# luoao-kddi/SCP

Hardware: AMD Instinct MI355X
Metric: KITTI frames/sec encode (SCP-EHEM, level 16) + bpp match vs ref (higher is better)
Workload: dtype f32 (dense layers and attention as bf16x3 split on bf16 MFMA, feature kNN as f16x3 split on f16 MFMA, fp32 accumulate; position kNN / CDF in fp32); 1 GPU; SCP-EHEM KITTI-like synthetic 120k-pt frames, --spher --mullevel lidar_level=16 (BASELINE.json configs[2]), seeded random weights; nodes_per_frame=577403, windows_per_frame=100, frames_per_gpu=46, frames_in_flight=4, frames_per_launch_sequence=1, transform=host-numpy on a prefetch thread (strict identity: the reference's integers), parallelism=frame-sharded x1, rank_cores=256, rank_cores_pinned=False

## Files before the change

scp_amd/build.py:

```python
import os
import subprocess
import sys

HERE = os.path.dirname(os.path.abspath(__file__))
CSRC = os.path.join(HERE, "csrc")
LIB = os.path.join(HERE, "libscp_hip.so")
SOURCES = ["api.cpp", "geom.hip", "sort_u64.hip", "cdf.hip", "rangecoder.cpp", "legacy_octree.cpp",
           "knn.hip", "edge.hip", "attn.hip", "octattn.hip", "octattn_f16.hip", "octattn_embed.hip", "octattn_rowinv.hip", "gemm.hip", "gemm_split.hip", "rowchain.hip", "fused.hip", "metrics.hip", "plan.hip"]
HIPCC = os.environ.get("HIPCC", "/opt/rocm/bin/hipcc")
FLAGS = ["-O3", "--offload-arch=gfx950", "-fPIC", "-std=c++17", "-Wall", "-Wno-unused-function",
         "-Wno-unused-result", "-fvisibility=hidden", "-x", "hip"]


EXTRA = {"geom.hip": ["-ffp-contract=off"], "knn.hip": ["-ffp-contract=off"], "cdf.hip": ["-ffp-contract=off"],
         "edge.hip": ["-ffp-contract=off"], "metrics.hip": ["-ffp-contract=off"], "octattn_embed.hip": ["-ffp-contract=off"],
         "octattn_rowinv.hip": ["-ffp-contract=off"]}
if os.environ.get("SCP_ATTN_DEFS"):
    EXTRA["attn.hip"] = os.environ["SCP_ATTN_DEFS"].split()
if os.environ.get("SCP_KNN_DEFS"):
    EXTRA["knn.hip"] = EXTRA["knn.hip"] + os.environ["SCP_KNN_DEFS"].split()
if os.environ.get("SCP_RC_DEFS"):
    EXTRA["rowchain.hip"] = os.environ["SCP_RC_DEFS"].split()


def _stale(target, deps):
    if not os.path.exists(target):
        return True
    t = os.path.getmtime(target)
    return any(os.path.getmtime(d) > t for d in deps)


def build(force=False, verbose=False):
    srcs = [os.path.join(CSRC, s) for s in SOURCES if os.path.exists(os.path.join(CSRC, s))]
    hdrs = [os.path.join(CSRC, f) for f in os.listdir(CSRC) if f.endswith(".h")] + [os.path.join(HERE, "..", "include", "scp.h")]
    objs = []
    os.makedirs(os.path.join(CSRC, "build"), exist_ok=True)
    procs = []
    for s in srcs:
        o = os.path.join(CSRC, "build", os.path.basename(s) + ".o")
        objs.append(o)
        cmd = [HIPCC] + FLAGS + EXTRA.get(os.path.basename(s), []) + ["-c", s, "-o", o]
        stamp, line = o + ".cmd", " ".join(cmd)
        same_cmd = os.path.exists(stamp) and open(stamp).read() == line
        if force or not same_cmd or _stale(o, [s] + hdrs):
            for stale in (stamp, o):
                if os.path.exists(stale):
                    os.remove(stale)
            if verbose:
                print(" ".join(cmd), file=sys.stderr)
            procs.append((s, subprocess.Popen(cmd), stamp, line))
    bad = []
    for s, p, stamp, line in procs:
        if p.wait() != 0:
            bad.append(s)
            continue
        with open(stamp, "w") as f:
            f.write(line)
    if bad:
        raise RuntimeError("hipcc failed for: " + ", ".join(bad))
    if force or procs or _stale(LIB, objs):
        cmd = [HIPCC, "--offload-arch=gfx950", "-shared", "-fPIC", "-o", LIB] + objs
        if verbose:
            print(" ".join(cmd), file=sys.stderr)
        subprocess.check_call(cmd)
    return LIB


if __name__ == "__main__":
    print(build(force="--force" in sys.argv, verbose=True))
```

scp_amd/csrc/rowchain.hip:

```cpp
#include <stdlib.h>
#include "scp_internal.h"

typedef __bf16 rbf16x8 __attribute__((ext_vector_type(8)));
typedef float rf32x16 __attribute__((ext_vector_type(16)));
typedef float rf32x4 __attribute__((ext_vector_type(4)));
typedef int ri32x4 __attribute__((ext_vector_type(4)));
typedef __attribute__((address_space(3))) void *rc_lds_ptr_t;
typedef const __attribute__((address_space(1))) void *rc_glb_ptr_t;

#define RC_ROWS 128
#define RC_SLOT 32768
#define RC_RING (4 * RC_SLOT)
#define RC_BOUNCE 4096
#define RC_OFF_BOUNCE RC_RING
#define RC_OFF_BIAS (RC_RING + 4 * RC_BOUNCE)
#define RC_LDS (RC_OFF_BIAS + 16384)

__device__ __forceinline__ void rc_dma16(const void *g, char *l) {
    __builtin_amdgcn_global_load_lds((rc_glb_ptr_t)g, (rc_lds_ptr_t)l, 16, 0, 0);
}

typedef float rf32x2 __attribute__((ext_vector_type(2)));
typedef __bf16 rbf16x2 __attribute__((ext_vector_type(2)));
typedef unsigned ru32x4 __attribute__((ext_vector_type(4)));
typedef unsigned ru32x2 __attribute__((ext_vector_type(2)));
__device__ __forceinline__ unsigned rc_pack2(float a, float b) {
    const rf32x2 v = {a, b};
    return __builtin_bit_cast(unsigned, __builtin_convertvector(v, rbf16x2));
}
__device__ __forceinline__ void rc_split2(float a, float b, unsigned &hi, unsigned &lo) {
    asm volatile("" : "+v"(a), "+v"(b));
    hi = rc_pack2(a, b);
    lo = rc_pack2(a - __builtin_bit_cast(float, hi << 16), b - __builtin_bit_cast(float, hi & 0xffff0000u));
}
__device__ __forceinline__ void rc_split8(const float *f, rbf16x8 &hi, rbf16x8 &lo) {
    ru32x4 h, l;
#pragma unroll
    for (int i = 0; i < 4; ++i) { unsigned a, b; rc_split2(f[2 * i], f[2 * i + 1], a, b); h[i] = a; l[i] = b; }
    hi = __builtin_bit_cast(rbf16x8, h);
    lo = __builtin_bit_cast(rbf16x8, l);
}

struct RcLane {
    int lane, col, h, w;
    int frag;
    int rg;
};

__device__ __forceinline__ RcLane rc_lane() {
    RcLane L;
    const int tid = threadIdx.x;
    L.lane = tid & 63; L.col = L.lane & 31; L.h = L.lane >> 5;
    L.w = __builtin_amdgcn_readfirstlane(tid >> 6);
    L.frag = (L.col & 15) * 64 + ((L.h ^ ((L.col >> 2) & 3)) << 4);
    L.rg = L.col >> 4;
    return L;
}

__device__ __forceinline__ void rc_issue_rowchunk(const RcLane &L, const __bf16 *Whi, const __bf16 *Wlo, int g, char *slot) {
#pragma unroll
    for (int j = 0; j < 4; ++j) {
        const int p = L.w + 4 * j;
        const int64_t off = ((int64_t)g * 16 + p) * 512 + L.lane * 8;
        rc_dma16(Whi + off, slot + p * 1024);
        rc_dma16(Wlo + off, slot + 16384 + p * 1024);
    }
}

__device__ __forceinline__ void rc_issue_kchunk(const RcLane &L, const __bf16 *Whi, const __bf16 *Wlo, int c, int nks, char *slot) {
#pragma unroll
    for (int j = 0; j < 4; ++j) {
        const int p = L.w + 4 * j;
        const int64_t off = ((int64_t)p * nks + c) * 512 + L.lane * 8;
        rc_dma16(Whi + off, slot + p * 1024);
        rc_dma16(Wlo + off, slot + 16384 + p * 1024);
    }
}

__device__ __forceinline__ rbf16x8 rc_frag_rowchunk(const RcLane &L, const char *slot, int plane, int s) {
    return *(const rbf16x8 *)(slot + plane * 16384 + (L.rg * 8 + (s >> 1)) * 1024 + (L.frag ^ ((s & 1) << 5)));
}

__device__ __forceinline__ rbf16x8 rc_frag_kchunk(const RcLane &L, const char *slot, int plane, int b, int t) {
    return *(const rbf16x8 *)(slot + plane * 16384 + (2 * b + L.rg) * 1024 + (L.frag ^ (t << 5)));
}

#define RC_DS_READ4_WAIT(d0, a0, o0, d1, a1, o1, d2, a2, o2, d3, a3, o3)                                                              \
    asm volatile("ds_read_b128 %0, %4 offset:%8\n\tds_read_b128 %1, %5 offset:%9\n\tds_read_b128 %2, %6 offset:%10\n\t"                   \
                 "ds_read_b128 %3, %7 offset:%11\n\ts_waitcnt lgkmcnt(0)"                                                              \
                 : "=&v"(d0), "=&v"(d1), "=&v"(d2), "=&v"(d3) : "v"(a0), "v"(a1), "v"(a2), "v"(a3), "n"(o0), "n"(o1), "n"(o2), "n"(o3) : "memory")
#define RC_DS_READ(dst, addr, off) asm volatile("ds_read_b128 %0, %1 offset:%2" : "=v"(dst) : "v"(addr), "n"(off) : "memory")

__device__ __forceinline__ void rc_mfma3x2(rf32x16 &c0, rf32x16 &c1, const rbf16x8 &a0h, const rbf16x8 &a0l, const rbf16x8 &a1h,
                                           const rbf16x8 &a1l, const rbf16x8 &bh, const rbf16x8 &bl) {
    c0 = __builtin_amdgcn_mfma_f32_32x32x16_bf16(a0l, bh, c0, 0, 0, 0);
    c1 = __builtin_amdgcn_mfma_f32_32x32x16_bf16(a1l, bh, c1, 0, 0, 0);
    c0 = __builtin_amdgcn_mfma_f32_32x32x16_bf16(a0h, bl, c0, 0, 0, 0);
    c1 = __builtin_amdgcn_mfma_f32_32x32x16_bf16(a1h, bl, c1, 0, 0, 0);
    c0 = __builtin_amdgcn_mfma_f32_32x32x16_bf16(a0h, bh, c0, 0, 0, 0);
    c1 = __builtin_amdgcn_mfma_f32_32x32x16_bf16(a1h, bh, c1, 0, 0, 0);
}

__device__ __forceinline__ void rc_store_block(const RcLane &L, char *bounce, const rf32x4 v[4], __amdgpu_buffer_rsrc_t rs, int ldo_bytes, int voff,
                                               int ch0) {
#pragma unroll
    for (int q = 0; q < 4; ++q)
        *(rf32x4 *)(bounce + L.col * 128 + (((2 * q + L.h) ^ (L.col & 7)) << 4)) = v[q];
    asm volatile("s_waitcnt lgkmcnt(0)" ::: "memory");
    rf32x4 y[4];
#pragma unroll
    for (int it = 0; it < 4; ++it) {
        const int rho = 8 * it + (L.lane >> 3), kap = L.lane & 7;
        y[it] = *(const rf32x4 *)(bounce + rho * 128 + ((kap ^ (rho & 7)) << 4));
    }
#pragma unroll
    for (int it = 0; it < 4; ++it) __builtin_amdgcn_raw_buffer_store_b128(__builtin_bit_cast(ri32x4, y[it]), rs, voff, it * 8 * ldo_bytes + ch0 * 4, 0);
    asm volatile("s_waitcnt lgkmcnt(0)" ::: "memory");
}

__device__ __forceinline__ void rc_ln_stats(const float *v , float eps, float &mean, float &rstd) {
    float s = 0.f;
#pragma unroll
    for (int i = 0; i < 128; i += 4) s += (v[i] + v[i + 1]) + (v[i + 2] + v[i + 3]);
    s += __shfl_xor(s, 32);
    mean = s * (1.0f / 256.0f);
    float q = 0.f;
#pragma unroll
    for (int i = 0; i < 128; ++i) { const float d = v[i] - mean; q += d * d; }
    q += __shfl_xor(q, 32);
    rstd = rsqrtf(q * (1.0f / 256.0f) + eps);
}

struct RcLnLinArgs {
    const float *x; int64_t ldx;
    const float *valid;
    const __bf16 *Whi, *Wlo;
    const float *bias, *wbeta;
    float *out; int64_t ldo;
    int M, N;
    float eps;
    int probe;
    unsigned long long *dbg;
    __bf16 *planes; int64_t plane_bytes; int nq;
    int ngroups;
};

#define RC_DS_WRITE(addr, val, off) asm volatile("ds_write_b128 %0, %1 offset:%2" :: "v"(addr), "v"(val), "n"(off) : "memory")

#define RC_SB __builtin_amdgcn_sched_barrier(0)
#ifndef RC_SKEW
#define RC_SKEW 0
#endif
#if RC_SKEW > 0
#define RC_STEP_BARRIER(WAITS, w)                                                                                                          \
    do {                                                                                                                                   \
        int _rc_n;                                                                                                                         \
        asm volatile("s_waitcnt " WAITS "\n\ts_barrier\n\ts_mov_b32 %0, %1\n\ts_cmp_eq_u32 %0, 0\n\ts_cbranch_scc1 .Lrcskew_done%=\n"          \
                     ".Lrcskew_loop%=:\n\ts_nop 7\n\ts_sub_u32 %0, %0, 1\n\ts_cmp_lg_u32 %0, 0\n\ts_cbranch_scc1 .Lrcskew_loop%=\n"              \
                     ".Lrcskew_done%=:"                                                                                                   \
                     : "=&s"(_rc_n) : "s"((w) * RC_SKEW) : "memory", "scc");                                                                \
    } while (0)
#else
#ifdef RC_PROBE_NOBAR
#define RC_STEP_BARRIER(WAITS, w) asm volatile("s_waitcnt " WAITS ::: "memory")
#else
#define RC_STEP_BARRIER(WAITS, w) asm volatile("s_waitcnt " WAITS "\n\ts_barrier" ::: "memory")
#endif
#endif
#ifdef RC_PROBE_NODMA
#define RC_PROBE_DMA_ON 0
#else
#define RC_PROBE_DMA_ON 1
#endif
#ifdef RC_PROBE_NOFRAG
#define RC_PROBE_FRAG_ON 0
#else
#define RC_PROBE_FRAG_ON 1
#endif
#ifdef RC_DMA_SPREAD
#define RC_DMA_P(s, gap) ((s) < 4 ? 2 * (s) + ((gap) == 3) : (s) + 4)
#define RC_DMA_HERE(s, gap) (((s) < 4 && ((gap) == 1 || (gap) == 3)) || ((s) >= 4 && (s) < 12 && (gap) == 1))
#define RC_DMA_SLOT(s, gap) (RC_DMA_P(s, gap) >> 3)
#define RC_DMA_IDX(s, gap) ((RC_DMA_P(s, gap) >> 1) & 3)
#define RC_DMA_PLANE(s, gap) (RC_DMA_P(s, gap) & 1)
#else
#define RC_DMA_HERE(s, gap) ((s) < 8 && ((gap) == 1 || (gap) == 3))
#define RC_DMA_SLOT(s, gap) ((s) >> 2)
#define RC_DMA_IDX(s, gap) ((s) & 3)
#define RC_DMA_PLANE(s, gap) ((gap) >> 1)
#endif
#ifdef RC_WAIT0
#define RC_FRAG_WAIT() asm volatile("s_waitcnt lgkmcnt(0)" ::: "memory")
#else
#define RC_FRAG_WAIT() asm volatile("s_waitcnt lgkmcnt(3)" ::: "memory")
#endif
#ifndef RC_STORE_AUX
#define RC_STORE_AUX 0
#endif
template <bool LOADX, int PROBE, bool SWAP = false, bool NSWAP = false>
__device__ __forceinline__ void rc_ll_step(const RcLane &L, const RcLnLinArgs &a, char *smem, int half, rf32x16 &c0, rf32x16 &c1,
                                           rf32x16 &p0, rf32x16 &p1, const rbf16x8 (&Xh)[16], const rbf16x8 (&Xl)[16], int g_next,
                                           __amdgpu_buffer_rsrc_t rs_prev, int voff, int ldo_bytes, int ch0_prev, const unsigned (&bw)[4],
                                           unsigned br, const float *xsrc, float (&v)[128], rbf16x8 (&A)[2][4], const float *tb_next, unsigned long long *st,
                                           __amdgpu_buffer_rsrc_t wr_hi, __amdgpu_buffer_rsrc_t wr_lo, const float *sbn = nullptr, unsigned maskh = 0) {
    const unsigned ab = (unsigned)(uintptr_t)(rc_lds_ptr_t)(smem + half * (2 * RC_SLOT)) + L.rg * 8192;
    const unsigned ad0 = ab + L.frag, ad1 = ab + (L.frag ^ 32);
    const unsigned an0 = (unsigned)(uintptr_t)(rc_lds_ptr_t)(smem + (half ^ 1) * (2 * RC_SLOT)) + L.rg * 8192 + L.frag;
    char *nxt = smem + (half ^ 1) * (2 * RC_SLOT);
    rf32x4 rd[4];
    unsigned long long ts0 = 0;
    if (st) ts0 = __builtin_amdgcn_s_memtime();
#pragma unroll
    for (int s = 0; s < 16; ++s) {
        if (st && (s == 1 || s == 8 || s == 15)) { const unsigned long long t = __builtin_amdgcn_s_memtime(); st[s == 1 ? 0 : s == 8 ? 1 : 2] += t - ts0; ts0 = t; }
        if (s == 15) {
            asm volatile("s_waitcnt lgkmcnt(0)" ::: "memory");
            if (PROBE) RC_STEP_BARRIER("vmcnt(0)", L.w);
            else if (LOADX) RC_STEP_BARRIER("vmcnt(24)", L.w);
            else RC_STEP_BARRIER("vmcnt(8)", L.w);
            if (st) { const unsigned long long t = __builtin_amdgcn_s_memtime(); st[3] += t - ts0; ts0 = t; }
        }
        RC_SB;
        const int nb = (s + 1) & 1, ns = (s + 1) & 15;
        const unsigned ra = (ns & 1) ? ad1 : ad0;
#pragma unroll
        for (int gap = 0; gap < 6; ++gap) {
            if (gap < 4) { RC_FRAG_WAIT(); RC_SB; }
#define RC_LL_MFMA(c, wf, xf) c = SWAP ? __builtin_amdgcn_mfma_f32_32x32x16_bf16(xf, wf, c, 0, 0, 0) : __builtin_amdgcn_mfma_f32_32x32x16_bf16(wf, xf, c, 0, 0, 0)
// ... 1261 lines not shown
            const rf32x4 v0 = *(const rf32x4 *)(q0 + 16 * s), v1 = *(const rf32x4 *)(q0 + 16 * s + 4);
            const float f[8] = {v0[0], v0[1], v0[2], v0[3], v1[0], v1[1], v1[2], v1[3]};
            rc_split8(f, Xh[s], Xl[s]);
        }
        RC_LAYER3(0)
        to_frags();
        RC_LAYER3(1)
        to_frags();
        const int kap = L.lane & 7;
        float *orow[4];
#pragma unroll
        for (int it = 0; it < 4; ++it) {
            const int r = m0 + 32 * L.w + 8 * it + (L.lane >> 3);
            const int64_t o = r < a.M ? (a.out_map ? a.out_map[r] : (int64_t)r) : -1;
            orow[it] = o >= 0 ? a.out + o * a.ldo + 4 * kap : nullptr;
        }
        auto store_block = [&](const rf32x16 &c, int ch0) {
#pragma unroll
            for (int q = 0; q < 4; ++q) {
                rf32x4 v;
#pragma unroll
                for (int u = 0; u < 4; ++u) v[u] = c[4 * q + u];
                *(rf32x4 *)(bounce + L.col * 128 + (((2 * q + L.h) ^ (L.col & 7)) << 4)) = v;
            }
            asm volatile("s_waitcnt lgkmcnt(0)" ::: "memory");
            rf32x4 y[4];
#pragma unroll
            for (int it = 0; it < 4; ++it) {
                const int rho = 8 * it + (L.lane >> 3);
                y[it] = *(const rf32x4 *)(bounce + rho * 128 + ((kap ^ (rho & 7)) << 4));
            }
            asm volatile("s_waitcnt lgkmcnt(0)" ::: "memory");
#pragma unroll
            for (int it = 0; it < 4; ++it)
                if (orow[it] && ch0 + 4 * kap < a.N) *(rf32x4 *)(orow[it] + ch0) = y[it];
        };
        for (int g = 0; g < 4; ++g) {
            RC_BIAS3(2)
            RC_STEP3()
            store_block(c0, 64 * g);
            store_block(c1, 64 * g + 32);
        }
#undef RC_LAYER3
#undef RC_BIAS3
#undef RC_STEP3
    }
    SCP_WAIT_DMA(0);
}

extern "C" SCP_API double scp_gelu_prescale(void) { return (double)SCP_GELU_S; }

static int rc_ll_groups(int ntiles, int nsteps, int ncu) {
    static int on = -1;
    if (on < 0) { const char *e = getenv("SCP_RC_GROUPS"); on = (e && e[0] == '0') ? 0 : 1; }
    int best = 1;
    if (on)
        for (int g = 2; g <= nsteps / 2; ++g)
            if ((nsteps / 2) % g == 0 && (int64_t)ntiles * g <= ncu) best = g;
    return best;
}

static unsigned long long *g_rc_dbg = nullptr;
extern "C" SCP_API int scp_rc_debug_buffer(unsigned long long *dev_buf) { g_rc_dbg = dev_buf; return SCP_OK; }

static int g_rc_num_cu = 0, g_rc_grid = 0;
static int g_rc_wide = -2;
static int rc_wide_mode() {
    if (g_rc_wide == -2) { const char *e = getenv("SCP_RC_WIDE"); g_rc_wide = e ? atoi(e) : -1; if (g_rc_wide < -1 || g_rc_wide > 1) g_rc_wide = -1; }
    return g_rc_wide;
}
extern "C" SCP_API int scp_rc_set_wide(int32_t mode) { g_rc_wide = (mode < -1 || mode > 1) ? -1 : mode; return SCP_OK; }
extern "C" SCP_API int scp_rc_set_grid(int32_t workgroups) { g_rc_grid = workgroups > 0 ? workgroups : 0; return SCP_OK; }
static int rc_num_cu() {
    if (g_rc_grid) return g_rc_grid;
    if (!g_rc_num_cu) {
        int dev = 0;
        hipDeviceProp_t p;
        if (hipGetDevice(&dev) != hipSuccess || hipGetDeviceProperties(&p, dev) != hipSuccess) return 256;
        g_rc_num_cu = p.multiProcessorCount > 0 ? p.multiProcessorCount : 256;
    }
    return g_rc_num_cu;
}

extern "C" SCP_API int scp_swin_ln_linear(const float *x, int64_t ldx, const float *valid, const void *Whi, const void *Wlo, const float *bias,
                                          const float *wbeta, float eps, float *out, int64_t ldo, int32_t M, int32_t N, void *stream) {
    if (!x || !Whi || !Wlo || !out || M <= 0 || N <= 0 || (N & 127) || N > 1024 || ldx < 256 || (ldx & 3) || ldo < N || (ldo & 3) ||
        (((uintptr_t)x | (uintptr_t)out | (uintptr_t)Whi | (uintptr_t)Wlo) & 15) || (int64_t)RC_ROWS * ldo * 4 > 0x7fffffffLL)
        return SCP_EINVAL;
    static bool configured = false;
    if (!configured) {
        HIP_TRY(hipFuncSetAttribute((const void *)rc_ln_linear_kernel<0>, hipFuncAttributeMaxDynamicSharedMemorySize, RC_LDS));
        configured = true;
    }
    RcLnLinArgs a;
    a.x = x; a.ldx = ldx; a.valid = valid; a.Whi = (const __bf16 *)Whi; a.Wlo = (const __bf16 *)Wlo; a.bias = bias; a.wbeta = wbeta;
    a.out = out; a.ldo = ldo; a.M = M; a.N = N; a.eps = eps;
    a.planes = nullptr; a.plane_bytes = 0; a.nq = 0;
    { static int pr = -1; if (pr < 0) { const char *e = getenv("SCP_RC_PROBE"); pr = e ? atoi(e) : 0; } a.probe = pr; }
    if (a.probe) { const char *e = getenv("SCP_RC_PROBE"); a.probe = e ? atoi(e) : 0; }
    a.dbg = g_rc_dbg;
    const int ntiles = (M + RC_ROWS - 1) / RC_ROWS;
    const int ncu = rc_num_cu();
    SCP_PROF(SCP_PROF_LN_LINEAR, stream, 2.0 * M * 256.0 * N);
    a.ngroups = rc_ll_groups(ntiles, N / 64, ncu);
    hipLaunchKernelGGL(rc_ln_linear_kernel<0>, dim3((unsigned)(a.ngroups > 1 ? ntiles * a.ngroups : (ntiles < ncu ? ntiles : ncu))), dim3(256), RC_LDS, (hipStream_t)stream, a);
    LAUNCH_CHECK();
    return SCP_OK;
}

extern "C" SCP_API int scp_swin_ln_qkv(const float *x, int64_t ldx, const float *valid, const void *Whi, const void *Wlo, const float *bias,
                                       const float *wbeta, float eps, float *q, int64_t ldq, void *planes, int64_t Tp, int32_t M, int32_t N, void *stream) {
    if (!x || !Whi || !Wlo || !planes || M <= 0 || (M & 127) || (N != 768 && N != 512) || (N == 768 && (!q || ldq < 256 || (ldq & 3))) || ldx < 256 ||
        (ldx & 3) || Tp < M || (Tp & 31) || (((uintptr_t)x | (uintptr_t)q | (uintptr_t)Whi | (uintptr_t)Wlo | (uintptr_t)planes) & 15) ||
        (q && (int64_t)RC_ROWS * ldq * 4 > 0x7fffffffLL) || 4 * Tp * 512 > 0x7fffffffLL)
        return SCP_EINVAL;
    static bool configured = false;
    if (!configured) {
        HIP_TRY(hipFuncSetAttribute((const void *)rc_ln_linear_kernel<0, true>, hipFuncAttributeMaxDynamicSharedMemorySize, RC_LDS));
        configured = true;
    }
    RcLnLinArgs a;
    a.x = x; a.ldx = ldx; a.valid = valid; a.Whi = (const __bf16 *)Whi; a.Wlo = (const __bf16 *)Wlo; a.bias = bias; a.wbeta = wbeta;
    a.out = q; a.ldo = q ? ldq : 256; a.M = M; a.N = N; a.eps = eps; a.probe = 0; a.dbg = nullptr;
    a.planes = (__bf16 *)planes; a.plane_bytes = Tp * 512; a.nq = N / 64 - 8;
    const int ntiles = M / RC_ROWS, ncu = rc_num_cu();
    SCP_PROF(SCP_PROF_LN_LINEAR, stream, 2.0 * M * 256.0 * N);
    a.ngroups = rc_ll_groups(ntiles, N / 64, ncu);
    hipLaunchKernelGGL((rc_ln_linear_kernel<0, true>), dim3((unsigned)(a.ngroups > 1 ? ntiles * a.ngroups : (ntiles < ncu ? ntiles : ncu))), dim3(256), RC_LDS, (hipStream_t)stream, a);
    LAUNCH_CHECK();
    return SCP_OK;
}

extern "C" SCP_API int scp_swin_post_attn(const void *Ohi, const void *Olo, int64_t ldo_in, const float *x, int64_t ldx, const void *W, const float *bp,
                                          const float *b1, const float *b2, float eps, float *out, int64_t ldc, int32_t M, const int32_t *tile_list,
                                          int32_t n_tiles, void *stream) {
    if (!Ohi || !Olo || !x || !W || !bp || !b1 || !b2 || !out || M <= 0 || (tile_list && (n_tiles <= 0 || n_tiles > (M + RC_ROWS - 1) / RC_ROWS)) || ldo_in < 256 || (ldo_in & 7) || ldx < 256 || (ldx & 3) || ldc < 256 ||
        (ldc & 3) || (((uintptr_t)Ohi | (uintptr_t)Olo | (uintptr_t)x | (uintptr_t)out | (uintptr_t)W) & 15) ||
        (int64_t)RC_ROWS * ldc * 4 > 0x7fffffffLL)
        return SCP_EINVAL;
    static bool configured = false;
    if (!configured) {
        HIP_TRY(hipFuncSetAttribute((const void *)rc_post_attn_kernel, hipFuncAttributeMaxDynamicSharedMemorySize, RC_LDS));
        HIP_TRY(hipFuncSetAttribute((const void *)rc_post_attn_wide_kernel, hipFuncAttributeMaxDynamicSharedMemorySize, RC_LDS));
        configured = true;
    }
    RcPostArgs a;
    a.Ohi = (const __bf16 *)Ohi; a.Olo = (const __bf16 *)Olo; a.ldo_in = ldo_in; a.x = x; a.ldx = ldx; a.W = W;
    a.bp = bp; a.b1 = b1; a.b2 = b2; a.out = out; a.ldc = ldc; a.M = M; a.eps = eps;
    a.dbg = g_rc_dbg;
    { const char *e = getenv("SCP_RC_DUMP"); a.dbg_mode = e ? atoi(e) : 0; }
    a.tile_list = tile_list; a.n_list = tile_list ? n_tiles : 0;
    const int ntiles = tile_list ? n_tiles : (M + RC_ROWS - 1) / RC_ROWS;
    const int ncu = rc_num_cu();
    SCP_PROF(SCP_PROF_POST_ATTN, stream, 2.0 * (tile_list ? (double)n_tiles * RC_ROWS : (double)M) * (256.0 * 256.0 + 2.0 * 256.0 * 1024.0));
    if (rc_wide_mode() == 1 || (rc_wide_mode() < 0 && !g_rc_dbg && !a.dbg_mode && 4 * (int64_t)ntiles <= (int64_t)ncu)) {
        const int items = 4 * ntiles;
        hipLaunchKernelGGL(rc_post_attn_wide_kernel, dim3((unsigned)(items < 2 * ncu ? items : 2 * ncu)), dim3(256), RC_LDS, (hipStream_t)stream, a);
        LAUNCH_CHECK();
        return SCP_OK;
    }
    hipLaunchKernelGGL(rc_post_attn_kernel, dim3((unsigned)(ntiles < ncu ? ntiles : ncu)), dim3(256), RC_LDS, (hipStream_t)stream, a);
    LAUNCH_CHECK();
    return SCP_OK;
}

extern "C" SCP_API int64_t scp_swin_post_attn_weight_bytes(void) { return 2 * (int64_t)RC_W_PLANE; }

extern "C" SCP_API int scp_geo_edge_mlps(const float *pos1, int64_t ld1, const float *pos2, int64_t ld2, const float *pos3, int64_t ld3, const void *W,
                                         const float *bias, float *out, int64_t ldo, int32_t M, void *stream) {
    if (!pos1 || !pos2 || !pos3 || !W || !bias || !out || M <= 0 || ld1 < 64 || ld2 < 128 || ld3 < 256 || ((ld1 | ld2 | ld3) & 3) || ldo < 128 || (ldo & 3) ||
        (((uintptr_t)pos1 | (uintptr_t)pos2 | (uintptr_t)pos3 | (uintptr_t)out | (uintptr_t)W) & 15) || (int64_t)RC_ROWS * ldo * 4 > 0x7fffffffLL)
        return SCP_EINVAL;
    static bool configured = false;
    if (!configured) {
        HIP_TRY(hipFuncSetAttribute((const void *)rc_edge_mlp_kernel, hipFuncAttributeMaxDynamicSharedMemorySize, RC_LDS));
        configured = true;
    }
    RcEdgeArgs a;
    a.p1 = pos1; a.p2 = pos2; a.p3 = pos3; a.ld1 = ld1; a.ld2 = ld2; a.ld3 = ld3; a.W = W; a.bias = bias; a.out = out; a.ldo = ldo; a.M = M;
    const int ntiles = (M + RC_ROWS - 1) / RC_ROWS, ncu = rc_num_cu();
    SCP_PROF(SCP_PROF_EDGE_MLP, stream, 2.0 * M * (448.0 * 256 + 2.0 * 256 * 256 + 512.0 * 256 + 256.0 * 256 + 256.0 * 128));
    hipLaunchKernelGGL(rc_edge_mlp_kernel, dim3((unsigned)(ntiles < ncu ? ntiles : ncu)), dim3(256), RC_LDS, (hipStream_t)stream, a);
    LAUNCH_CHECK();
    return SCP_OK;
}

extern "C" SCP_API int scp_mlp3_rows(const float *x, int64_t ldx, int64_t n_src, const int64_t *in_map, const void *W, const float *bias, float *out, int64_t ldo,
                                     const int64_t *out_map, int32_t M, int32_t N, void *stream) {
    if (!x || !W || !bias || !out || M <= 0 || n_src <= 0 || N <= 0 || N > 256 || (N & 3) || ldx < 256 || (ldx & 3) || ldo < N || (ldo & 3) ||
        (((uintptr_t)x | (uintptr_t)out | (uintptr_t)W) & 15))
        return SCP_EINVAL;
    static bool configured = false;
    if (!configured) {
        HIP_TRY(hipFuncSetAttribute((const void *)rc_mlp3_kernel, hipFuncAttributeMaxDynamicSharedMemorySize, RC_LDS));
        configured = true;
    }
    RcMlp3Args a;
    a.x = x; a.ldx = ldx; a.in_map = in_map; a.n_src = n_src; a.W = W; a.bias = bias; a.out = out; a.ldo = ldo; a.out_map = out_map; a.M = M; a.N = N;
    const int ntiles = (M + RC_ROWS - 1) / RC_ROWS, ncu = rc_num_cu();
    SCP_PROF(SCP_PROF_MLP3, stream, 2.0 * M * 3.0 * 256.0 * 256.0);
    hipLaunchKernelGGL(rc_mlp3_kernel, dim3((unsigned)(ntiles < ncu ? ntiles : ncu)), dim3(256), RC_LDS, (hipStream_t)stream, a);
    LAUNCH_CHECK();
    return SCP_OK;
}

extern "C" SCP_API int scp_swin_merge(const float *x, int64_t ldx, int64_t n_src, const int64_t *ia, const int64_t *ib, const void *W, const float *wbeta,
                                      float eps, float *out, int64_t ldo, int32_t M, void *stream) {
    if (!x || !ia || !ib || !W || !out || M <= 0 || n_src <= 0 || ldx < 256 || (ldx & 3) || ldo < 256 || (ldo & 3) ||
        (((uintptr_t)x | (uintptr_t)out | (uintptr_t)W) & 15) || (int64_t)RC_ROWS * ldo * 4 > 0x7fffffffLL)
// ... 15 lines not shown
```

Measured before the change: 15.61 frames/s.

## Add two-workgroup-per-CU LayerNorm+linear kernel with smaller weight ring

Adds a new fused LayerNorm + bf16x3 projection kernel (ln2_proj_kernel) whose LDS footprint fits under 80 KiB, so two workgroups can share a CU. It streams weights in quarter chunks through a three-slot buffer-load-to-LDS ring and prefetches A fragments one step ahead. It is dispatched for the QKV and plain ln_linear paths when the tile count is large relative to the CU count. It also moves shared helpers into a common header. The aim is better latency hiding through higher occupancy, at the cost of smaller per-CU weight staging and more register pressure from launch_bounds(256,2).

```diff
diff --git a/scp_amd/build.py b/scp_amd/build.py
--- a/scp_amd/build.py
+++ b/scp_amd/build.py
@@ -6,7 +6,7 @@
 CSRC = os.path.join(HERE, "csrc")
 LIB = os.path.join(HERE, "libscp_hip.so")
 SOURCES = ["api.cpp", "geom.hip", "sort_u64.hip", "cdf.hip", "rangecoder.cpp", "legacy_octree.cpp",
-           "knn.hip", "edge.hip", "attn.hip", "octattn.hip", "octattn_f16.hip", "octattn_embed.hip", "octattn_rowinv.hip", "gemm.hip", "gemm_split.hip", "rowchain.hip", "fused.hip", "metrics.hip", "plan.hip"]
+           "knn.hip", "edge.hip", "attn.hip", "octattn.hip", "octattn_f16.hip", "octattn_embed.hip", "octattn_rowinv.hip", "gemm.hip", "gemm_split.hip", "rowchain.hip", "lnlin2.hip", "fused.hip", "metrics.hip", "plan.hip"]
 HIPCC = os.environ.get("HIPCC", "/opt/rocm/bin/hipcc")
 FLAGS = ["-O3", "--offload-arch=gfx950", "-fPIC", "-std=c++17", "-Wall", "-Wno-unused-function",
          "-Wno-unused-result", "-fvisibility=hidden", "-x", "hip"]
@@ -21,6 +21,7 @@
     EXTRA["knn.hip"] = EXTRA["knn.hip"] + os.environ["SCP_KNN_DEFS"].split()
 if os.environ.get("SCP_RC_DEFS"):
     EXTRA["rowchain.hip"] = os.environ["SCP_RC_DEFS"].split()
+EXTRA["lnlin2.hip"] = EXTRA.get("rowchain.hip", [])
 
 
 def _stale(target, deps):
diff --git a/scp_amd/csrc/lnlin2.hip b/scp_amd/csrc/lnlin2.hip
--- /dev/null
+++ b/scp_amd/csrc/lnlin2.hip
@@ -0,0 +1,278 @@
+#include <stdlib.h>
+#include <type_traits>
+#include "rc_common.h"
+
+#define L2_Q 16384
+#define L2_OFF_BOUNCE (3 * L2_Q)
+#define L2_OFF_BIAS (L2_OFF_BOUNCE + 4 * RC_BOUNCE)
+#define L2_LDS (L2_OFF_BIAS + 8192)
+static_assert(L2_LDS <= 80 * 1024, "two workgroups per CU: at most half of the 160 KiB");
+#define L2_LDS_ONE (160 * 1024)
+
+__device__ __forceinline__ void l2_issue(const RcLane &L, __amdgpu_buffer_rsrc_t wr_hi, __amdgpu_buffer_rsrc_t wr_lo, int j, int qt, char *dst) {
+#pragma unroll
+    for (int i = 0; i < 4; ++i) {
+        const int b = i >> 1, plane = i & 1;
+        const int soff = ((2 * j + b) * 16 + (L.w >> 1) * 8 + qt * 2 + (L.w & 1)) * 1024;
+        __builtin_amdgcn_raw_ptr_buffer_load_lds(plane ? wr_lo : wr_hi, (rc_lds_ptr_t)(dst + (L.w + 4 * i) * 1024), 16, L.lane * 16, soff, 0, 0);
+    }
+}
+
+#define L2_READ4(d0, d1, d2, d3, addr, o0, o1, o2, o3)                                                                                  \
+    asm volatile("ds_read_b128 %0, %4 offset:%5\n\tds_read_b128 %1, %4 offset:%6\n\tds_read_b128 %2, %4 offset:%7\n\t"                      \
+                 "ds_read_b128 %3, %4 offset:%8\n\ts_waitcnt lgkmcnt(0)"                                                                  \
+                 : "=&v"(d0), "=&v"(d1), "=&v"(d2), "=&v"(d3) : "v"(addr), "n"(o0), "n"(o1), "n"(o2), "n"(o3) : "memory")
+#define L2_READ4_AHEAD(d0, d1, d2, d3, addr, o0, o1, o2, o3)                                                                            \
+    asm volatile("ds_read_b128 %0, %4 offset:%5\n\tds_read_b128 %1, %4 offset:%6\n\tds_read_b128 %2, %4 offset:%7\n\t"                      \
+                 "ds_read_b128 %3, %4 offset:%8"                                                                                         \
+                 : "=&v"(d0), "=&v"(d1), "=&v"(d2), "=&v"(d3) : "v"(addr), "n"(o0), "n"(o1), "n"(o2), "n"(o3) : "memory")
+#define L2_WAIT4(d0, d1, d2, d3) asm volatile("s_waitcnt lgkmcnt(0)" : "+v"(d0), "+v"(d1), "+v"(d2), "+v"(d3) :: "memory")
+#define L2_TOP(N) asm volatile("s_waitcnt vmcnt(" #N ") lgkmcnt(0)\n\ts_barrier" ::: "memory")
+
+template <bool SWAP, int Q>
+__device__ __forceinline__ void l2_quarter(unsigned ad0, unsigned ad1, rf32x16 &c0, rf32x16 &c1, const rbf16x8 (&Xh)[16], const rbf16x8 (&Xl)[16]) {
+#define L2_MFMA(c, wf, xf) c = SWAP ? __builtin_amdgcn_mfma_f32_32x32x16_bf16(xf, wf, c, 0, 0, 0) : __builtin_amdgcn_mfma_f32_32x32x16_bf16(wf, xf, c, 0, 0, 0)
+#define L2_FRAGS(M, A, ad, s) M(A[1], A[3], A[0], A[2], ad, 4096 + ((s) >> 1) * 1024, 12288 + ((s) >> 1) * 1024, ((s) >> 1) * 1024, 8192 + ((s) >> 1) * 1024)
+    rbf16x8 A[2][4];
+    L2_FRAGS(L2_READ4, A[0], ad0, 0);
+#pragma unroll
+    for (int s = 0; s < 4; ++s) {
+        const int k = 4 * Q + s, n = (s + 1) & 1;
+        if (s < 3) {
+            if (n) L2_FRAGS(L2_READ4_AHEAD, A[1], ad1, s + 1);
+            else L2_FRAGS(L2_READ4_AHEAD, A[0], ad0, s + 1);
+        }
+        __builtin_amdgcn_sched_barrier(0);
+        L2_MFMA(c0, A[s & 1][1], Xh[k]);
+        L2_MFMA(c1, A[s & 1][3], Xh[k]);
+        L2_MFMA(c0, A[s & 1][0], Xl[k]);
+        L2_MFMA(c1, A[s & 1][2], Xl[k]);
+        L2_MFMA(c0, A[s & 1][0], Xh[k]);
+        L2_MFMA(c1, A[s & 1][2], Xh[k]);
+        __builtin_amdgcn_sched_barrier(0);
+        if (s < 3) L2_WAIT4(A[n][0], A[n][1], A[n][2], A[n][3]);
+    }
+#undef L2_FRAGS
+#undef L2_MFMA
+}
+
+__device__ __forceinline__ unsigned l2_split_pair(float x0, float x1, int plane) {
+    const unsigned hh = rc_pack2(x0, x1);
+    return plane ? rc_pack2(x0 - __builtin_bit_cast(float, hh << 16), x1 - __builtin_bit_cast(float, hh & 0xffff0000u)) : hh;
+}
+
+__device__ __forceinline__ void l2_store_k(const RcLane &L, char *bounce, const rf32x16 &c0, const rf32x16 &c1, __amdgpu_buffer_rsrc_t prs, int kvoff,
+                                           int pbytes, int head) {
+    ri32x4 y[2][4];
+    int col = L.col;
+    asm volatile("" : "+v"(col));
+#pragma unroll
+    for (int plane = 0; plane < 2; ++plane) {
+#pragma unroll
+        for (int b = 0; b < 2; ++b)
+#pragma unroll
+            for (int q = 0; q < 4; ++q) {
+                const rf32x16 &c = b ? c1 : c0;
+                *(ru32x2 *)(bounce + col * 128 + (((4 * b + q) ^ (col & 7)) << 4) + 8 * L.h) =
+                    (ru32x2){l2_split_pair(c[4 * q], c[4 * q + 1], plane), l2_split_pair(c[4 * q + 2], c[4 * q + 3], plane)};
+            }
+#pragma unroll
+        for (int it = 0; it < 4; ++it) y[plane][it] = *(const ri32x4 *)(bounce + it * 1024 + L.lane * 16);
+    }
+#pragma unroll
+    for (int plane = 0; plane < 2; ++plane)
+#pragma unroll
+        for (int it = 0; it < 4; ++it)
+            __builtin_amdgcn_raw_buffer_store_b128(y[plane][it], prs, kvoff, it * 8 * 512 + head * 128 + plane * pbytes, 0);
+    asm volatile("s_waitcnt lgkmcnt(0)" ::: "memory");
+}
+
+__device__ __forceinline__ void l2_store_v(const RcLane &L, char *bounce, const rf32x16 &c0, const rf32x16 &c1, __amdgpu_buffer_rsrc_t prs, int vblk,
+                                           int pbytes, int head) {
+    ri32x4 y[2][4];
+    int col = L.col;
+    asm volatile("" : "+v"(col));
+#pragma unroll
+    for (int plane = 0; plane < 2; ++plane) {
+#pragma unroll
+        for (int b = 0; b < 2; ++b)
+#pragma unroll
+            for (int cc = 0; cc < 2; ++cc) {
+                const rf32x16 &c = b ? c1 : c0;
+                const int d = col + 32 * b, R = d >> 1, sl = (d & 1) * 4 + 2 * cc + L.h;
+                *(ru32x4 *)(bounce + R * 128 + ((sl ^ (R & 7)) << 4)) =
+                    (ru32x4){l2_split_pair(c[8 * cc], c[8 * cc + 1], plane), l2_split_pair(c[8 * cc + 2], c[8 * cc + 3], plane),
+                             l2_split_pair(c[8 * cc + 4], c[8 * cc + 5], plane), l2_split_pair(c[8 * cc + 6], c[8 * cc + 7], plane)};
+            }
+#pragma unroll
+        for (int it = 0; it < 4; ++it) y[plane][it] = *(const ri32x4 *)(bounce + it * 1024 + L.lane * 16);
+    }
+#pragma unroll
+    for (int plane = 0; plane < 2; ++plane)
+#pragma unroll
+        for (int it = 0; it < 4; ++it)
+            __builtin_amdgcn_raw_buffer_store_b128(y[plane][it], prs, L.lane * 16, it * 1024 + (vblk + head) * 4096 + (2 + plane) * pbytes, 0);
+    asm volatile("s_waitcnt lgkmcnt(0)" ::: "memory");
+}
+
+template <bool KV>
+__global__ __launch_bounds__(256, 2) void ln2_proj_kernel(const RcLnLinArgs a) {
+    extern __shared__ __attribute__((aligned(1024))) char smem[];
+    const RcLane L = rc_lane();
+    const int ntiles = (a.M + RC_ROWS - 1) / RC_ROWS;
+    const int nsteps = a.N >> 6;
+    const int nq = KV ? a.nq : nsteps;
+    char *bounce = smem + L2_OFF_BOUNCE + L.w * RC_BOUNCE;
+    const unsigned ab = (unsigned)(uintptr_t)(rc_lds_ptr_t)smem + L.rg * 2048;
+    const unsigned af0 = ab + L.frag, af1 = ab + (L.frag ^ 32);
+    const unsigned asb = (unsigned)(uintptr_t)(rc_lds_ptr_t)(smem + L2_OFF_BIAS);
+    const int ldo_bytes = (int)(a.ldo * 4);
+    const int voff = (32 * L.w + (L.lane >> 3)) * ldo_bytes + (L.lane & 7) * 16;
+    const int pbytes = (int)a.plane_bytes;
+    const __amdgpu_buffer_rsrc_t prs = __builtin_amdgcn_make_buffer_rsrc((void *)a.planes, 0, (KV && !(a.probe & 1)) ? (int)(4 * a.plane_bytes) : 0, 0x00020000);
+    const bool dma = !(a.probe & 2);
+
+    const int wbytes = ((a.N + 255) & ~255) * 512;
+    const __amdgpu_buffer_rsrc_t wr_hi = __builtin_amdgcn_make_buffer_rsrc((void *)a.Whi, 0, wbytes, 0x00020000);
+    const __amdgpu_buffer_rsrc_t wr_lo = __builtin_amdgcn_make_buffer_rsrc((void *)a.Wlo, 0, wbytes, 0x00020000);
+
+    float *sb = (float *)(smem + L2_OFF_BIAS), *sbw = sb + 1024;
+    for (int i = threadIdx.x; i < a.N; i += 256) {
+        const float b = a.bias ? a.bias[i] : 0.f;
+        sb[i] = b; sbw[i] = b + (a.wbeta ? a.wbeta[i] : 0.f);
+    }
+    __syncthreads();
+    int slot = 0;
+    if (dma) { l2_issue(L, wr_hi, wr_lo, 0, 0, smem); l2_issue(L, wr_hi, wr_lo, 0, 1, smem + L2_Q); }
+    for (int tile = blockIdx.x; tile < ntiles; tile += (int)gridDim.x) {
+        const int m0 = tile * RC_ROWS;
+        const int row = m0 + 32 * L.w + L.col;
+        const int rowc = row < a.M ? row : a.M - 1;
+        float keep = (row < a.M) ? 1.0f : 0.0f;
+        if (a.valid) keep *= a.valid[rowc];
+        rbf16x8 Xh[16], Xl[16];
+        {
+            float v[128];
+            const float *src = a.x + (int64_t)((a.probe & 4) ? (rowc & 127) % a.M : rowc) * a.ldx + 8 * L.h;
+#pragma unroll
+            for (int s = 0; s < 16; ++s) {
+                const rf32x4 q0 = *(const rf32x4 *)(src + 16 * s), q1 = *(const rf32x4 *)(src + 16 * s + 4);
+#pragma unroll
+                for (int u = 0; u < 4; ++u) { v[8 * s + u] = q0[u]; v[8 * s + 4 + u] = q1[u]; }
+            }
+            float mean, rstd;
+            rc_ln_stats(v, a.eps, mean, rstd);
+            const float sc = rstd * keep;
+#pragma unroll
+            for (int s = 0; s < 16; ++s) {
+                float f[8];
+#pragma unroll
+                for (int i = 0; i < 8; ++i) f[i] = (v[8 * s + i] - mean) * sc;
+                rc_split8(f, Xh[s], Xl[s]);
+            }
+        }
+        const bool kept = keep != 0.f;
+        const int64_t rows_left = (int64_t)a.M - m0;
+        const int64_t span = (rows_left < RC_ROWS ? rows_left : RC_ROWS) * a.ldo * 4;
+        const __amdgpu_buffer_rsrc_t rs = __builtin_amdgcn_make_buffer_rsrc(a.out + (int64_t)m0 * a.ldo, 0, (a.probe & 1) ? 0 : (int)span, 0x00020000);
+        const unsigned kmask = (unsigned)__builtin_amdgcn_ballot_w64(kept);
+        const unsigned maskh = kmask >> (4 * L.h);
+        const int kvoff = (m0 + 32 * L.w + (L.lane >> 3)) * 512 + (L.lane & 7) * 16;
+        const int vblk = ((m0 >> 5) + L.w) * 4;
+
+        const unsigned atb = asb + (kept ? 4096 : 0) + 16 * L.h, atv = asb + 4 * L.col;
+        rf32x16 c0, c1;
+        auto bias_start = [&](int j) {
+            if (KV && j >= nq + 4) {
+                float bb[2], bwv[2];
+                const unsigned ad = atv + 256 * j;
+                asm volatile("ds_read_b32 %0, %4\n\tds_read_b32 %1, %4 offset:128\n\tds_read_b32 %2, %4 offset:4096\n\tds_read_b32 %3, %4 offset:4224\n\t"
+                             "s_waitcnt lgkmcnt(0)" : "=&v"(bb[0]), "=&v"(bb[1]), "=&v"(bwv[0]), "=&v"(bwv[1]) : "v"(ad) : "memory");
+#pragma unroll
+                for (int blk = 0; blk < 2; ++blk) {
+                    rf32x16 &c = blk ? c1 : c0;
+#pragma unroll
+                    for (int r = 0; r < 16; ++r) c[r] = ((maskh >> (8 * (r >> 2) + (r & 3))) & 1u) ? bwv[blk] : bb[blk];
+                }
+            } else {
+                const unsigned ad = atb + 256 * j;
+                rf32x4 t[2][4];
+                L2_READ4(t[0][0], t[0][1], t[0][2], t[0][3], ad, 0, 32, 64, 96);
+                L2_READ4(t[1][0], t[1][1], t[1][2], t[1][3], ad, 128, 160, 192, 224);
+#pragma unroll
+                for (int q = 0; q < 4; ++q)
+#pragma unroll
+                    for (int u = 0; u < 4; ++u) { c0[4 * q + u] = t[0][q][u]; c1[4 * q + u] = t[1][q][u]; }
+            }
+        };
+        bias_start(0);
+        SCP_WAIT_DMA(0);
+        auto steps = [&](auto sw, int ja, int jb) {
+        constexpr bool SW = decltype(sw)::value;
+        for (int j = ja; j < jb; ++j) {
+            const int jn = j + 1 < nsteps ? j + 1 : 0;
+#define L2_QUARTER(Q, N)                                                                                                                \
+            {                                                                                                                           \
+                L2_TOP(N);                                                                                                              \
+                const int sl2 = slot == 0 ? 2 : slot - 1;                    \
+                if (dma) l2_issue(L, wr_hi, wr_lo, Q < 2 ? j : jn, (Q + 2) & 3, smem + sl2 * L2_Q);                                       \
+                __builtin_amdgcn_sched_barrier(0);                                                                                      \
+                const unsigned a0 = af0 + slot * L2_Q, a1 = af1 + slot * L2_Q;                                                          \
+                l2_quarter<SW, Q>(a0, a1, c0, c1, Xh, Xl);                                                                              \
+                slot = slot == 2 ? 0 : slot + 1;                                                                                        \
+            }
+            L2_QUARTER(0, 12)
+            L2_QUARTER(1, 12)
+            L2_QUARTER(2, 4)
+            L2_QUARTER(3, 4)
+#undef L2_QUARTER
+            __builtin_amdgcn_sched_barrier(0);
+            if (!SW && j < nq) {
+#pragma unroll
+                for (int blk = 0; blk < 2; ++blk) {
+                    rf32x4 o[4];
+#pragma unroll
+                    for (int q = 0; q < 4; ++q)
+#pragma unroll
+                        for (int u = 0; u < 4; ++u) o[q][u] = (blk ? c1 : c0)[4 * q + u];
+                    rc_store_block(L, bounce, o, rs, ldo_bytes, voff, 64 * j + 32 * blk);
+                }
+            } else if (!SW) {
+                l2_store_k(L, bounce, c0, c1, prs, kvoff, pbytes, j - nq);
+            } else {
+                l2_store_v(L, bounce, c0, c1, prs, vblk, pbytes, j - nq - 4);
+            }
+            if (j + 1 < nsteps) bias_start(jn);
+        }
+        };
+        if (KV) { steps(std::false_type(), 0, nq + 4); steps(std::true_type(), nq + 4, nsteps); }
+        else steps(std::false_type(), 0, nsteps);
+    }
+    SCP_WAIT_DMA(0);
+}
+
+int scp_lnlin2_mode() {
+    static int mode = -1;
+    if (mode < 0) { const char *e = getenv("SCP_LNLIN"); mode = e ? atoi(e) : 0; if (mode < 0 || mode > 2) mode = 0; }
+    return mode;
+}
+
+int scp_lnlin2_launch(RcLnLinArgs a, bool kv, int ncu, hipStream_t stream) {
+    static int one = -1, probe = -1;
+    if (one < 0) { const char *e = getenv("SCP_LNLIN_ONE"); one = (e && e[0] == '1') ? 1 : 0; }
+    if (probe < 0) { const char *e = getenv("SCP_RC_PROBE"); probe = e ? atoi(e) : 0; }
+    static bool configured = false;
+    if (!configured) {
+        HIP_TRY(hipFuncSetAttribute((const void *)ln2_proj_kernel<false>, hipFuncAttributeMaxDynamicSharedMemorySize, one ? L2_LDS_ONE : L2_LDS));
+        HIP_TRY(hipFuncSetAttribute((const void *)ln2_proj_kernel<true>, hipFuncAttributeMaxDynamicSharedMemorySize, one ? L2_LDS_ONE : L2_LDS));
+        configured = true;
+    }
+    a.ngroups = 1; a.probe = probe; a.dbg = nullptr;
+    const int ntiles = (a.M + RC_ROWS - 1) / RC_ROWS;
+    const int wgs = (one ? 1 : 2) * ncu;
+    const dim3 grid((unsigned)(ntiles < wgs ? ntiles : wgs));
+    if (kv) hipLaunchKernelGGL(ln2_proj_kernel<true>, grid, dim3(256), one ? L2_LDS_ONE : L2_LDS, stream, a);
+    else hipLaunchKernelGGL(ln2_proj_kernel<false>, grid, dim3(256), one ? L2_LDS_ONE : L2_LDS, stream, a);
+    LAUNCH_CHECK();
+    return SCP_OK;
+}
diff --git a/scp_amd/csrc/rc_common.h b/scp_amd/csrc/rc_common.h
--- /dev/null
+++ b/scp_amd/csrc/rc_common.h
@@ -0,0 +1,100 @@
+#pragma once
+#include "scp_internal.h"
+
+typedef __bf16 rbf16x8 __attribute__((ext_vector_type(8)));
+typedef float rf32x16 __attribute__((ext_vector_type(16)));
+typedef float rf32x4 __attribute__((ext_vector_type(4)));
+typedef int ri32x4 __attribute__((ext_vector_type(4)));
+typedef __attribute__((address_space(3))) void *rc_lds_ptr_t;
+typedef const __attribute__((address_space(1))) void *rc_glb_ptr_t;
+
+#define RC_ROWS 128
+#define RC_BOUNCE 4096
+
+__device__ __forceinline__ void rc_dma16(const void *g, char *l) {
+    __builtin_amdgcn_global_load_lds((rc_glb_ptr_t)g, (rc_lds_ptr_t)l, 16, 0, 0);
+}
+
+typedef float rf32x2 __attribute__((ext_vector_type(2)));
+typedef __bf16 rbf16x2 __attribute__((ext_vector_type(2)));
+typedef unsigned ru32x4 __attribute__((ext_vector_type(4)));
+typedef unsigned ru32x2 __attribute__((ext_vector_type(2)));
+__device__ __forceinline__ unsigned rc_pack2(float a, float b) {
+    const rf32x2 v = {a, b};
+    return __builtin_bit_cast(unsigned, __builtin_convertvector(v, rbf16x2));
+}
+__device__ __forceinline__ void rc_split2(float a, float b, unsigned &hi, unsigned &lo) {
+    asm volatile("" : "+v"(a), "+v"(b));
+    hi = rc_pack2(a, b);
+    lo = rc_pack2(a - __builtin_bit_cast(float, hi << 16), b - __builtin_bit_cast(float, hi & 0xffff0000u));
+}
+__device__ __forceinline__ void rc_split8(const float *f, rbf16x8 &hi, rbf16x8 &lo) {
+    ru32x4 h, l;
+#pragma unroll
+    for (int i = 0; i < 4; ++i) { unsigned a, b; rc_split2(f[2 * i], f[2 * i + 1], a, b); h[i] = a; l[i] = b; }
+    hi = __builtin_bit_cast(rbf16x8, h);
+    lo = __builtin_bit_cast(rbf16x8, l);
+}
+
+struct RcLane {
+    int lane, col, h, w;
+    int frag;
+    int rg;
+};
+
+__device__ __forceinline__ RcLane rc_lane() {
+    RcLane L;
+    const int tid = threadIdx.x;
+    L.lane = tid & 63; L.col = L.lane & 31; L.h = L.lane >> 5;
+    L.w = __builtin_amdgcn_readfirstlane(tid >> 6);
+    L.frag = (L.col & 15) * 64 + ((L.h ^ ((L.col >> 2) & 3)) << 4);
+    L.rg = L.col >> 4;
+    return L;
+}
+
+__device__ __forceinline__ void rc_store_block(const RcLane &L, char *bounce, const rf32x4 v[4], __amdgpu_buffer_rsrc_t rs, int ldo_bytes, int voff,
+                                               int ch0) {
+#pragma unroll
+    for (int q = 0; q < 4; ++q)
+        *(rf32x4 *)(bounce + L.col * 128 + (((2 * q + L.h) ^ (L.col & 7)) << 4)) = v[q];
+    asm volatile("s_waitcnt lgkmcnt(0)" ::: "memory");
+    rf32x4 y[4];
+#pragma unroll
+    for (int it = 0; it < 4; ++it) {
+        const int rho = 8 * it + (L.lane >> 3), kap = L.lane & 7;
+        y[it] = *(const rf32x4 *)(bounce + rho * 128 + ((kap ^ (rho & 7)) << 4));
+    }
+#pragma unroll
+    for (int it = 0; it < 4; ++it) __builtin_amdgcn_raw_buffer_store_b128(__builtin_bit_cast(ri32x4, y[it]), rs, voff, it * 8 * ldo_bytes + ch0 * 4, 0);
+    asm volatile("s_waitcnt lgkmcnt(0)" ::: "memory");
+}
+
+__device__ __forceinline__ void rc_ln_stats(const float *v , float eps, float &mean, float &rstd) {
+    float s = 0.f;
+#pragma unroll
+    for (int i = 0; i < 128; i += 4) s += (v[i] + v[i + 1]) + (v[i + 2] + v[i + 3]);
+    s += __shfl_xor(s, 32);
+    mean = s * (1.0f / 256.0f);
+    float q = 0.f;
+#pragma unroll
+    for (int i = 0; i < 128; ++i) { const float d = v[i] - mean; q += d * d; }
+    q += __shfl_xor(q, 32);
+    rstd = rsqrtf(q * (1.0f / 256.0f) + eps);
+}
+
+struct RcLnLinArgs {
+    const float *x; int64_t ldx;
+    const float *valid;
+    const __bf16 *Whi, *Wlo;
+    const float *bias, *wbeta;
+    float *out; int64_t ldo;
+    int M, N;
+    float eps;
+    int probe;
+    unsigned long long *dbg;
+    __bf16 *planes; int64_t plane_bytes; int nq;
+    int ngroups;
+};
+
+int scp_lnlin2_mode();
+int scp_lnlin2_launch(RcLnLinArgs a, bool kv, int ncu, hipStream_t stream);
diff --git a/scp_amd/csrc/rowchain.hip b/scp_amd/csrc/rowchain.hip
--- a/scp_amd/csrc/rowchain.hip
+++ b/scp_amd/csrc/rowchain.hip
@@ -1,61 +1,12 @@
 #include <stdlib.h>
 #include "scp_internal.h"
-
-typedef __bf16 rbf16x8 __attribute__((ext_vector_type(8)));
-typedef float rf32x16 __attribute__((ext_vector_type(16)));
-typedef float rf32x4 __attribute__((ext_vector_type(4)));
-typedef int ri32x4 __attribute__((ext_vector_type(4)));
-typedef __attribute__((address_space(3))) void *rc_lds_ptr_t;
-typedef const __attribute__((address_space(1))) void *rc_glb_ptr_t;
-
-#define RC_ROWS 128
+#include "rc_common.h"
+
 #define RC_SLOT 32768
 #define RC_RING (4 * RC_SLOT)
-#define RC_BOUNCE 4096
 #define RC_OFF_BOUNCE RC_RING
 #define RC_OFF_BIAS (RC_RING + 4 * RC_BOUNCE)
 #define RC_LDS (RC_OFF_BIAS + 16384)
-
-__device__ __forceinline__ void rc_dma16(const void *g, char *l) {
-    __builtin_amdgcn_global_load_lds((rc_glb_ptr_t)g, (rc_lds_ptr_t)l, 16, 0, 0);
-}
-
-typedef float rf32x2 __attribute__((ext_vector_type(2)));
-typedef __bf16 rbf16x2 __attribute__((ext_vector_type(2)));
-typedef unsigned ru32x4 __attribute__((ext_vector_type(4)));
-typedef unsigned ru32x2 __attribute__((ext_vector_type(2)));
-__device__ __forceinline__ unsigned rc_pack2(float a, float b) {
-    const rf32x2 v = {a, b};
-    return __builtin_bit_cast(unsigned, __builtin_convertvector(v, rbf16x2));
-}
-__device__ __forceinline__ void rc_split2(float a, float b, unsigned &hi, unsigned &lo) {
-    asm volatile("" : "+v"(a), "+v"(b));
-    hi = rc_pack2(a, b);
-    lo = rc_pack2(a - __builtin_bit_cast(float, hi << 16), b - __builtin_bit_cast(float, hi & 0xffff0000u));
-}
-__device__ __forceinline__ void rc_split8(const float *f, rbf16x8 &hi, rbf16x8 &lo) {
-    ru32x4 h, l;
-#pragma unroll
-    for (int i = 0; i < 4; ++i) { unsigned a, b; rc_split2(f[2 * i], f[2 * i + 1], a, b); h[i] = a; l[i] = b; }
-    hi = __builtin_bit_cast(rbf16x8, h);
-    lo = __builtin_bit_cast(rbf16x8, l);
-}
-
-struct RcLane {
-    int lane, col, h, w;
-    int frag;
-    int rg;
-};
-
-__device__ __forceinline__ RcLane rc_lane() {
-    RcLane L;
-    const int tid = threadIdx.x;
-    L.lane = tid & 63; L.col = L.lane & 31; L.h = L.lane >> 5;
-    L.w = __builtin_amdgcn_readfirstlane(tid >> 6);
-    L.frag = (L.col & 15) * 64 + ((L.h ^ ((L.col >> 2) & 3)) << 4);
-    L.rg = L.col >> 4;
-    return L;
-}
 
 __device__ __forceinline__ void rc_issue_rowchunk(const RcLane &L, const __bf16 *Whi, const __bf16 *Wlo, int g, char *slot) {
 #pragma unroll
@@ -101,49 +52,8 @@
     c1 = __builtin_amdgcn_mfma_f32_32x32x16_bf16(a1h, bh, c1, 0, 0, 0);
 }
 
-__device__ __forceinline__ void rc_store_block(const RcLane &L, char *bounce, const rf32x4 v[4], __amdgpu_buffer_rsrc_t rs, int ldo_bytes, int voff,
-                                               int ch0) {
-#pragma unroll
-    for (int q = 0; q < 4; ++q)
-        *(rf32x4 *)(bounce + L.col * 128 + (((2 * q + L.h) ^ (L.col & 7)) << 4)) = v[q];
-    asm volatile("s_waitcnt lgkmcnt(0)" ::: "memory");
-    rf32x4 y[4];
-#pragma unroll
-    for (int it = 0; it < 4; ++it) {
-        const int rho = 8 * it + (L.lane >> 3), kap = L.lane & 7;
-        y[it] = *(const rf32x4 *)(bounce + rho * 128 + ((kap ^ (rho & 7)) << 4));
-    }
-#pragma unroll
-    for (int it = 0; it < 4; ++it) __builtin_amdgcn_raw_buffer_store_b128(__builtin_bit_cast(ri32x4, y[it]), rs, voff, it * 8 * ldo_bytes + ch0 * 4, 0);
-    asm volatile("s_waitcnt lgkmcnt(0)" ::: "memory");
-}
-
-__device__ __forceinline__ void rc_ln_stats(const float *v , float eps, float &mean, float &rstd) {
-    float s = 0.f;
-#pragma unroll
-    for (int i = 0; i < 128; i += 4) s += (v[i] + v[i + 1]) + (v[i + 2] + v[i + 3]);
-    s += __shfl_xor(s, 32);
-    mean = s * (1.0f / 256.0f);
-    float q = 0.f;
-#pragma unroll
-    for (int i = 0; i < 128; ++i) { const float d = v[i] - mean; q += d * d; }
-    q += __shfl_xor(q, 32);
-    rstd = rsqrtf(q * (1.0f / 256.0f) + eps);
-}
-
-struct RcLnLinArgs {
-    const float *x; int64_t ldx;
-    const float *valid;
-    const __bf16 *Whi, *Wlo;
-    const float *bias, *wbeta;
-    float *out; int64_t ldo;
-    int M, N;
-    float eps;
-    int probe;
-    unsigned long long *dbg;
-    __bf16 *planes; int64_t plane_bytes; int nq;
-    int ngroups;
-};
+
+
 
 #define RC_DS_WRITE(addr, val, off) asm volatile("ds_write_b128 %0, %1 offset:%2" :: "v"(addr), "v"(val), "n"(off) : "memory")
 
@@ -1571,6 +1481,11 @@
     return g_rc_num_cu;
 }
 
+static bool rc_lnlin2_here(int ntiles, int ncu) {
+    const int mode = scp_lnlin2_mode();
+    return mode == 2 || (mode == 0 && 4 * (int64_t)ntiles >= 3 * (int64_t)ncu);
+}
+
 extern "C" SCP_API int scp_swin_ln_linear(const float *x, int64_t ldx, const float *valid, const void *Whi, const void *Wlo, const float *bias,
                                           const float *wbeta, float eps, float *out, int64_t ldo, int32_t M, int32_t N, void *stream) {
     if (!x || !Whi || !Wlo || !out || M <= 0 || N <= 0 || (N & 127) || N > 1024 || ldx < 256 || (ldx & 3) || ldo < N || (ldo & 3) ||
@@ -1591,6 +1506,7 @@
     const int ntiles = (M + RC_ROWS - 1) / RC_ROWS;
     const int ncu = rc_num_cu();
     SCP_PROF(SCP_PROF_LN_LINEAR, stream, 2.0 * M * 256.0 * N);
+    if (rc_lnlin2_here(ntiles, ncu)) return scp_lnlin2_launch(a, false, ncu, (hipStream_t)stream);
     a.ngroups = rc_ll_groups(ntiles, N / 64, ncu);
     hipLaunchKernelGGL(rc_ln_linear_kernel<0>, dim3((unsigned)(a.ngroups > 1 ? ntiles * a.ngroups : (ntiles < ncu ? ntiles : ncu))), dim3(256), RC_LDS, (hipStream_t)stream, a);
     LAUNCH_CHECK();
@@ -1614,6 +1530,7 @@
     a.planes = (__bf16 *)planes; a.plane_bytes = Tp * 512; a.nq = N / 64 - 8;
     const int ntiles = M / RC_ROWS, ncu = rc_num_cu();
     SCP_PROF(SCP_PROF_LN_LINEAR, stream, 2.0 * M * 256.0 * N);
+    if (rc_lnlin2_here(ntiles, ncu)) return scp_lnlin2_launch(a, true, ncu, (hipStream_t)stream);
     a.ngroups = rc_ll_groups(ntiles, N / 64, ncu);
     hipLaunchKernelGGL((rc_ln_linear_kernel<0, true>), dim3((unsigned)(a.ngroups > 1 ? ntiles * a.ngroups : (ntiles < ncu ? ntiles : ncu))), dim3(256), RC_LDS, (hipStream_t)stream, a);
     LAUNCH_CHECK();
```

Result: faster. 15.87 frames/s, median of 6 (+1.6%).
